# OpenHardware-Initiative/Drone-OA-IREE-ViT-Accelerator

Hardware: AMD Instinct MI355X
Metric: frames/s on ITAViTLSTM int8, 60x90 depth input (higher is better)
Workload: dtype int8+f32; 1 GPU; ITAViTLSTM int8 end-to-end forward (BASELINE config 4): 1024 synthetic 60x90 depth frames per GPU per step, LSTM state carried, velocity all-gather; frames_per_gpu=1024, global_batch=1024, parallelism=dp1, image_dtype=u8, weights=seed-0 synthetic QAT (tests/golden), gather_every=1, gather=none (one GPU), schedule=one stream

## Files before the change

### drone-oa-iree-vit-accelerator_amd/csrc/ita_lstm_head_kernel.h

```cpp
#pragma once
#include <cstddef>
#include "ita_f16x3_kernels.h"

__device__ __forceinline__ size_t ita_lstm_plane_index(int b, int k) {
  return ((size_t)(((b >> 5) * 4 + (k >> 6)) * 4 + ((k >> 4) & 3)) * 64 + ((k >> 3) & 1) * 32 + (b & 31)) * 8 + (k & 7);
}
__device__ __forceinline__ float lstm_sigmoid_fast(float x) {
  return __builtin_amdgcn_rcpf(1.0f + __builtin_amdgcn_exp2f(x * -1.44269504088896341f));
}
__device__ __forceinline__ float lstm_tanh_fast(float x) {
  return 1.0f - 2.0f * __builtin_amdgcn_rcpf(__builtin_amdgcn_exp2f(x * 2.88539008177792681f) + 1.0f);
}

__device__ __forceinline__ f32x16 mfma_f16x3(f32x16 acc, f16x8 wh, f16x8 wl, f16x8 xh, f16x8 xl) {
  acc = __builtin_amdgcn_mfma_f32_32x32x16_f16(wl, xh, acc, 0, 0, 0);
  acc = __builtin_amdgcn_mfma_f32_32x32x16_f16(wh, xl, acc, 0, 0, 0);
  return __builtin_amdgcn_mfma_f32_32x32x16_f16(wh, xh, acc, 0, 0, 0);
}
__device__ __forceinline__ void lstm_cell_fast(float gi, float gf, float gg, float go, float c_prev, float& c, float& h) {
  const float ig = lstm_sigmoid_fast(gi), fg = lstm_sigmoid_fast(gf), cg = lstm_tanh_fast(gg), og = lstm_sigmoid_fast(go);
  c = fmaf(fg, c_prev, ig * cg);
  h = og * lstm_tanh_fast(c);
}
__device__ __forceinline__ void split_f16x4(f32x4 x, f16x4& hi, f16x4& lo) {
#pragma unroll
  for (int j = 0; j < 4; ++j) {
    _Float16 a, b;
    split_f16(x[j], a, b);
    hi[j] = a;
    lo[j] = b;
  }
}
__device__ __forceinline__ f32x4 lstm_l0_extra(float dv, f32x4 q, int h, float& x4) {
  f32x4 x0 = {0.0f, 0.0f, 0.0f, 0.0f};
  x4 = 0.0f;
  if (h == 0) {
    x0 = (f32x4){dv / 10.0f, q.x, q.y, q.z};
    x4 = q.w;
  }
  return x0;
}
template <int NS>
__device__ __forceinline__ f32x4 sum_partials(const f32x4 (&pz)[NS]) {
  f32x4 ps = pz[0];
#pragma unroll
  for (int z = 1; z < NS; ++z) ps += pz[z];
  return ps;
}
__device__ __forceinline__ float lstm_sum4(const float (*part)[16][64], int e, int pl) {
  return ((part[0][e][pl] + part[1][e][pl]) + part[2][e][pl]) + part[3][e][pl];
}
template <class Live>
__device__ __forceinline__ void lstm_fc_rows(const float (*hs)[132], const float (*fw)[128], const float* fc_b, float* vel,
                                             size_t row0, int f0, int B, int tid, Live live) {
  if (tid < 96) {
    const int fr = tid / 3, o = tid - 3 * fr, b = f0 + fr;
    if (b < B && live(b)) {
      float acc = fc_b[o];
      for (int k = 0; k < 128; ++k) acc = fmaf(hs[fr][k], fw[o][k], acc);
      vel[(row0 + b) * 3 + o] = acc;
    }
  }
}

constexpr int ITA_HEAD_CNT_STRIDE = 64;
constexpr unsigned ITA_HEAD_ERR_TIMEOUT = 1;
constexpr unsigned long long ITA_HEAD_SPIN_TICKS = 200000000ull;
__device__ __forceinline__ void ita_store_sc1_f16x4(f16x4 v, __amdgpu_buffer_rsrc_t rsrc, int byte_off) {
  __builtin_amdgcn_raw_buffer_store_b64(__builtin_bit_cast(u32x2, v), rsrc, byte_off, 0, ITA_SC1);
}
__device__ __forceinline__ void ita_gather_h8(float hn, _Float16 (*pub)[32][8], int ef, int eu) {
  _Float16 x, y;
  split_f16(hn, x, y);
  pub[0][ef][eu] = x;
  pub[1][ef][eu] = y;
  __syncthreads();
}
__device__ __forceinline__ void ita_publish_h8(const _Float16 (*pub)[32][8], int r, __amdgpu_buffer_rsrc_t hi, int off_hi,
                                               __amdgpu_buffer_rsrc_t lo, int off_lo) {
  const f16x8 vh = *(const f16x8*)&pub[0][r][0], vl = *(const f16x8*)&pub[1][r][0];
  __builtin_amdgcn_raw_buffer_store_b128(__builtin_bit_cast(u32x4, vh), hi, off_hi, 0, ITA_SC1);
  __builtin_amdgcn_raw_buffer_store_b128(__builtin_bit_cast(u32x4, vl), lo, off_lo, 0, ITA_SC1);
}
__device__ __forceinline__ f16x8 ita_load_sc1_f16x8(__amdgpu_buffer_rsrc_t rsrc, int byte_off) {
  return __builtin_bit_cast(f16x8, __builtin_amdgcn_raw_buffer_load_b128(rsrc, byte_off, 0, ITA_SC1));
}
__device__ __forceinline__ f32x4 ita_load_sc1_f32x4(__amdgpu_buffer_rsrc_t rsrc, int byte_off) {
  return __builtin_bit_cast(f32x4, __builtin_amdgcn_raw_buffer_load_b128(rsrc, byte_off, 0, ITA_SC1));
}
__device__ __forceinline__ unsigned ita_head_arrive(unsigned* cnt, int ft, int tid) {
  asm volatile("s_waitcnt vmcnt(0)" ::: "memory");
  __syncthreads();
  unsigned prev = 0;
  if (tid == 0) prev = __hip_atomic_fetch_add(cnt + ft * ITA_HEAD_CNT_STRIDE, 1u, __ATOMIC_RELAXED, __HIP_MEMORY_SCOPE_AGENT);
  return prev;
}
__device__ __forceinline__ bool ita_head_poll(unsigned* cnt, unsigned target, unsigned* err) {
  const unsigned long long t0 = wall_clock64();
  while (__hip_atomic_load(cnt, __ATOMIC_RELAXED, __HIP_MEMORY_SCOPE_AGENT) < target) {
    if (wall_clock64() - t0 > ITA_HEAD_SPIN_TICKS) {
      __hip_atomic_fetch_or(err, ITA_HEAD_ERR_TIMEOUT, __ATOMIC_RELAXED, __HIP_MEMORY_SCOPE_AGENT);
      return false;
    }
    __builtin_amdgcn_s_sleep(2);
  }
  return true;
}


struct ItaLstmModelArgs {
  const float* part; float inv_fold_scale;
  const _Float16 *w0_hi, *w0_lo; float inv_wscale0;
  const float* bias0;
  const _Float16 *w1_hi, *w1_lo, *w2_hi, *w2_lo;
  float inv_wscale1, inv_wscale2;
  const float *bsum1, *bsum2;
};
struct ItaLstmHeadArgs {
  ItaLstmModelArgs m;
  const float *desvel, *quat;
  const float *h_in, *c_in;
  float *h_out, *c_out;
  size_t lstride;
  _Float16 *p1_hi, *p1_lo, *p2_hi, *p2_lo;
  const float *fc_w, *fc_b; float* vel;
  unsigned *cnt, *err;
  int B;
  const int* slots;
};
static_assert(sizeof(ItaLstmModelArgs) == 104 && offsetof(ItaLstmHeadArgs, desvel) == 104, "kernel-argument layout");

template <int NS>
__global__ __launch_bounds__(256, 2) void ita_lstm_head_kernel(const ItaLstmHeadArgs a) {
  __shared__ __attribute__((aligned(16))) float big[32 * 132 + 32 * 36];
  __shared__ __attribute__((aligned(16))) f16x8 hin[2][2][4][2][64];
  __shared__ __attribute__((aligned(16))) _Float16 pub[2][32][8];
  __shared__ unsigned flag;
  float (*hs)[132] = (float (*)[132])big;
  float (*pt)[36] = (float (*)[36])(big + 32 * 132);
  float (*part)[16][64] = (float (*)[16][64])big;
  const int tid = threadIdx.x, lane = tid & 63, wave = __builtin_amdgcn_readfirstlane(tid >> 6);
  const int ft = blockIdx.x >> 4, ut = blockIdx.x & 15, f0 = ft * 32;
  const int r = lane & 31, h = lane >> 5;
  const int B = a.B;
  const int ef = tid >> 3, eu = tid & 7;
  int rh[4], rb0 = min(f0 + r, B - 1), reb = min(f0 + ef, B - 1);
#pragma unroll
  for (int i = 0; i < 4; ++i) rh[i] = min(f0 + 2 * (4 * wave + i) + h, B - 1);
  if (a.slots) {
#pragma unroll
    for (int i = 0; i < 4; ++i) rh[i] = a.slots[rh[i]];
    rb0 = a.slots[rb0];
    reb = a.slots[reb];
  }

  f32x4 pz[NS];
#pragma unroll
  for (int z = 0; z < NS; ++z)
    pz[z] = *(const f32x4*)(a.m.part + ((size_t)z * B + min(f0 + 8 * wave + (lane >> 3), B - 1)) * 512 + ut * 32 + 4 * (lane & 7));
  f32x4 hv[4];
#pragma unroll
  for (int i = 0; i < 4; ++i) hv[i] = *(const f32x4*)(a.h_in + (size_t)rh[i] * 128 + 4 * r);
  const int b0 = f0 + r, u0 = ut * 8 + 4 * h;
  const size_t sb0 = (size_t)rb0;
  if (wave >= 2) {
    f32x4 hx[2][4][2];
#pragma unroll
    for (int l = 0; l < 2; ++l)
#pragma unroll
      for (int s = 0; s < 4; ++s) {
        const float* src = a.h_in + (l + 1) * a.lstride + sb0 * 128 + 64 * (wave - 2) + 16 * s + 8 * h;
        hx[l][s][0] = *(const f32x4*)src;
        hx[l][s][1] = *(const f32x4*)(src + 4);
      }
    __builtin_amdgcn_sched_barrier(0);
#pragma unroll
    for (int l = 0; l < 2; ++l)
#pragma unroll
      for (int s = 0; s < 4; ++s) {
        f16x8 xh, xl;
#pragma unroll
        for (int j = 0; j < 8; ++j) {
          _Float16 hi, lo;
          split_f16(hx[l][s][j >> 2][j & 3], hi, lo);
          xh[j] = hi;
          xl[j] = lo;
        }
        hin[l][wave - 2][s][0][lane] = xh;
        hin[l][wave - 2][s][1][lane] = xl;
      }
  }
  f16x8 wh[9], wl[9];
  f32x4 q = {0.0f, 0.0f, 0.0f, 0.0f}, ci0 = {0.0f, 0.0f, 0.0f, 0.0f}, bz[4];
  float dv = 0.0f;
  if (wave == 0) {
    const _Float16* wfr_hi = a.m.w0_hi + ((size_t)ut * 9 * 64 + lane) * 8;
    const _Float16* wfr_lo = a.m.w0_lo + ((size_t)ut * 9 * 64 + lane) * 8;
#pragma unroll
    for (int s = 0; s < 9; ++s) {
      wh[s] = *(const f16x8*)(wfr_hi + s * 512);
      wl[s] = *(const f16x8*)(wfr_lo + s * 512);
    }
    const int bc = min(b0, B - 1);
    q = *(const f32x4*)(a.quat + (size_t)bc * 4);
    dv = a.desvel[bc];
    ci0 = *(const f32x4*)(a.c_in + sb0 * 128 + u0);
#pragma unroll
    for (int gt = 0; gt < 4; ++gt) bz[gt] = *(const f32x4*)(a.m.bias0 + gt * 128 + u0);
  }
  const size_t wo = ((size_t)((ut * 4 + wave) * 4) * 64 + lane) * 8;
  f16x8 w1h[4], w1l[4];
#pragma unroll
  for (int s = 0; s < 4; ++s) {
    w1h[s] = *(const f16x8*)(a.m.w1_hi + wo + 512 * s);
    w1l[s] = *(const f16x8*)(a.m.w1_lo + wo + 512 * s);
  }
  const int eb = f0 + ef, un = ut * 8 + eu;
  const size_t esb = (size_t)reb;
  const float c1_prev = a.c_in[a.lstride + esb * 128 + un], c2_prev = a.c_in[2 * a.lstride + esb * 128 + un];
  float bs1[4], bs2[4];
#pragma unroll
  for (int gt = 0; gt < 4; ++gt) {
    bs1[gt] = a.m.bsum1[gt * 128 + un];
    bs2[gt] = a.m.bsum2[gt * 128 + un];
  }
  __builtin_amdgcn_sched_barrier(0);
  *(f32x4*)&pt[8 * wave + (lane >> 3)][4 * (lane & 7)] = sum_partials(pz);
#pragma unroll
  for (int i = 0; i < 4; ++i) *(f32x4*)&hs[2 * (4 * wave + i) + h][4 * r] = hv[i];
  __syncthreads();

  f32x4 hn0 = {0.0f, 0.0f, 0.0f, 0.0f};
  if (wave == 0) {
    f32x16 acc = {};
    float xlast1;
    const f32x4 xlast0 = lstm_l0_extra(dv, q, h, xlast1);
#pragma unroll
    for (int s = 0; s < 9; ++s) {
      f32x4 x0 = xlast0, x1 = {xlast1, 0.0f, 0.0f, 0.0f};
      if (s < 8) {
        x0 = *(const f32x4*)&hs[r][16 * s + 8 * h];
        x1 = *(const f32x4*)&hs[r][16 * s + 8 * h + 4];
      }
      f16x8 xh, xl;
#pragma unroll
      for (int j = 0; j < 8; ++j) {
        const float x = j < 4 ? x0[j & 3] : x1[j & 3];
        const _Float16 hi = (_Float16)x;
        xh[j] = hi;
        xl[j] = (_Float16)(x - (float)hi);
      }
      acc = mfma_f16x3(acc, wh[s], wl[s], xh, xl);
    }
    f32x4 cn;
#pragma unroll
    for (int q = 0; q < 4; ++q) {
      float g[4];
#pragma unroll
      for (int gt = 0; gt < 4; ++gt)
        g[gt] = (pt[r][gt * 8 + 4 * h + q] * a.m.inv_fold_scale + acc[4 * gt + q] * a.m.inv_wscale0) + bz[gt][q];
      float c, hn;
      lstm_cell_fast(g[0], g[1], g[2], g[3], ci0[q], c, hn);
      cn[q] = c;
      hn0[q] = hn;
    }
    if (b0 < B) *(f32x4*)(a.c_out + sb0 * 128 + u0) = cn;
    f16x4 x_hi, x_lo;
    split_f16x4(hn0, x_hi, x_lo);
    const int o0 = (int)ita_lstm_plane_index(b0, u0) * 2;
    ita_store_sc1_f16x4(x_hi, ita_rsrc(a.p1_hi), o0);
    ita_store_sc1_f16x4(x_lo, ita_rsrc(a.p1_lo), o0);
  }
  (void)ita_head_arrive(a.cnt, ft, tid);
  f16x8 w2h[4], w2l[4];
#pragma unroll
  for (int s = 0; s < 4; ++s) {
    w2h[s] = *(const f16x8*)(a.m.w2_hi + wo + 512 * s);
    w2l[s] = *(const f16x8*)(a.m.w2_lo + wo + 512 * s);
  }

#pragma unroll
  for (int l = 1; l <= 2; ++l) {
    if (tid == 0) flag = ita_head_poll(a.cnt + ft * ITA_HEAD_CNT_STRIDE, 16u * l, a.err) ? 1u : 0u;
    __syncthreads();
    if (!flag) return;
    if (l == 1 && wave == 0 && b0 < B) *(f32x4*)(a.h_out + sb0 * 128 + u0) = hn0;
    f16x8 fah[4], fal[4];
    if (wave < 2) {
      const int ao = (((ft * 4 + wave) * 4) * 64 + lane) * 16;
      const _Float16* ph = l == 1 ? a.p1_hi : a.p2_hi;
      const _Float16* pl = l == 1 ? a.p1_lo : a.p2_lo;
#pragma unroll
      for (int s = 0; s < 4; ++s) {
        fah[s] = ita_load_sc1_f16x8(ita_rsrc(ph), ao + 1024 * s);
        fal[s] = ita_load_sc1_f16x8(ita_rsrc(pl), ao + 1024 * s);
      }
    } else {
#pragma unroll
      for (int s = 0; s < 4; ++s) {
        fah[s] = hin[l - 1][wave - 2][s][0][lane];
        fal[s] = hin[l - 1][wave - 2][s][1][lane];
      }
    }
    f32x16 acc = {};
#pragma unroll
    for (int s = 0; s < 4; ++s) acc = mfma_f16x3(acc, l == 1 ? w1h[s] : w2h[s], l == 1 ? w1l[s] : w2l[s], fah[s], fal[s]);
#pragma unroll
    for (int e = 0; e < 16; ++e) part[wave][e][lane] = acc[e];
    __syncthreads();
    float gsum[4];
    const int pl = ef + 32 * (eu >> 2);
#pragma unroll
    for (int gte = 0; gte < 4; ++gte) gsum[gte] = lstm_sum4(part, 4 * gte + (eu & 3), pl);
    const float iws = l == 1 ? a.m.inv_wscale1 : a.m.inv_wscale2;
    const float* bs = l == 1 ? bs1 : bs2;
    const float gi = gsum[0] * iws + bs[0], gf = gsum[1] * iws + bs[1], gg = gsum[2] * iws + bs[2], go = gsum[3] * iws + bs[3];
    float c, hn;
    lstm_cell_fast(gi, gf, gg, go, l == 1 ? c1_prev : c2_prev, c, hn);
    const size_t so = l * a.lstride + esb * 128 + un;
    if (eb < B) {
      a.c_out[so] = c;
      if (l == 1) a.h_out[so] = hn;
      else
        __builtin_amdgcn_raw_buffer_store_b32(__builtin_bit_cast(unsigned, hn), ita_rsrc(a.h_out), (int)(so * 4), 0, ITA_SC1);
    }
    if (l == 1) {
      ita_gather_h8(hn, pub, ef, eu);
      if (wave == 0 && h == 0) {
        const int o = (int)ita_lstm_plane_index(f0 + r, ut * 8) * 2;
        ita_publish_h8(pub, r, ita_rsrc(a.p2_hi), o, ita_rsrc(a.p2_lo), o);
      }
    }
    const unsigned prev = ita_head_arrive(a.cnt, ft, tid);
    if (tid == 0 && l == 2) flag = prev == 47u ? 1u : 0u;
  }

  __syncthreads();
  if (!flag) return;
  if (tid == 0) __hip_atomic_store(a.cnt + ft * ITA_HEAD_CNT_STRIDE, 0u, __ATOMIC_RELAXED, __HIP_MEMORY_SCOPE_AGENT);
  float (*fw)[128] = (float (*)[128])(big + 32 * 132);
  int fro[4];
#pragma unroll
  for (int i = 0; i < 4; ++i) fro[i] = min(f0 + ((i * 256 + tid) >> 5), B - 1);
  if (a.slots) {
#pragma unroll
    for (int i = 0; i < 4; ++i) fro[i] = a.slots[fro[i]];
  }
  f32x4 hr[4];
#pragma unroll
  for (int i = 0; i < 4; ++i)
    hr[i] = ita_load_sc1_f32x4(ita_rsrc(a.h_out), (int)((2 * a.lstride + (size_t)fro[i] * 128 + 4 * (tid & 31)) * 4));
  const f32x4 wv = *(const f32x4*)(a.fc_w + 4 * min(tid, 95));
#pragma unroll
  for (int i = 0; i < 4; ++i) *(f32x4*)&hs[(i * 256 + tid) >> 5][4 * (tid & 31)] = hr[i];
  if (tid < 96) *(f32x4*)&fw[tid >> 5][4 * (tid & 31)] = wv;
  __syncthreads();
  lstm_fc_rows(hs, fw, a.fc_b, a.vel, 0, f0, B, tid, [](int) { return true; });
}
```

### drone-oa-iree-vit-accelerator_amd/csrc/ita_plugin.hip

```cpp
#include <hip/hip_runtime.h>

#include <algorithm>
#include <cstdio>
#include <cstdlib>
#include <cstring>
#include <mutex>
#include <string>
#include <atomic>
#include <thread>
#include <memory>
#include <type_traits>
#include <vector>

#include "../../include/ita_mi355x.h"
#include "../../include/ita_weights.h"
#include "../../include/ita_wire.h"
#include "ita_f16x3_kernels.h"
#include "ita_lstm_head_kernel.h"
#include "ita_lstm_seq_kernel.h"
#include "ita_f32_kernels.h"
#include "ita_int8_kernels.h"
#include "ita_stream_kernel.h"
#include "ita_long_attn_kernel.h"
#include "ita_long_stats_kernel.h"
// ... 1010 lines not shown
                                         (const float*)tp.row_max, (const float*)tp.row_sum, seq_len);
  });
}

}

int ita_mha_long_f32(ita_handle h, int layer, const float* x, float* y, int batch, int seq_len, void* stream) {
  if (int rc = check_layer_io(h, layer, x, y, batch)) return rc;
  return launch_long_f32(h, layer, x, y, false, batch, seq_len, (hipStream_t)stream);
}

int ita_mha_long_f32_taps(ita_handle h, int layer, const float* x, float* y, int batch, int seq_len,
                          const struct ita_mha_long_f32_taps* taps, void* stream) {
  if (int rc = check_layer_io(h, layer, x, y, batch)) return rc;
  const struct ita_mha_long_f32_taps none{};
  return launch_long_f32(h, layer, x, y, false, batch, seq_len, (hipStream_t)stream, taps ? taps : &none);
}

int ita_mha_long_f32_stats(ita_handle h, int layer, const float* x, int batch, int seq_len, float p_min,
                           const struct ita_mha_long_f32_stats* st, void* stream) {
  if (!h || !x || !st) return fail(ITA_ERR_INVALID_ARG, "null handle, x_dev or stats");
  if (!st->row_max && !st->row_sum && !st->row_gap && !st->row_nnz && !st->col_mass && !st->col_nnz)
    return fail(ITA_ERR_INVALID_ARG, "ita_mha_long_f32_stats: all six outputs are null");
  if (misaligned(st->row_max, 4) || misaligned(st->row_sum, 4) || misaligned(st->row_gap, 4) || misaligned(st->row_nnz, 4) ||
      misaligned(st->col_mass, 4) || misaligned(st->col_nnz, 4))
    return fail(ITA_ERR_INVALID_ARG, "every output must be 4-byte aligned");
  if (!(p_min > 0.0f && p_min <= 1.0f)) return fail(ITA_ERR_INVALID_ARG, "p_min must be in (0, 1]");
  if (int rc = check(h, batch)) return rc;
  if (layer < 0 || layer >= h->w.hdr.num_layers) return fail(ITA_ERR_INVALID_ARG, "bad layer");
  const Layer& L = h->w.layers[layer];
  hipStream_t s = (hipStream_t)stream;
  if (int rc = check_long_f32(L, batch, seq_len,
                              "this layer's attention is int8 (ITAW0001 / ITAW0002 blob): ita_mha_long_int8_stats reads it out")) return rc;
  const size_t nqt = (size_t)seq_len / 128, ntile = (size_t)batch * nqt;
  const size_t img = ntile * 2 * ItaLongF32Lds::UNIT, part = ntile * seq_len * 4;
  const bool cols = st->col_mass || st->col_nnz;
  if (int rc = ensure_long_f32_ws(h, 2 * img + (cols ? 2 * part : 0), s)) return rc;
  ItaLongF32Args a{};
  a.x = x;
  a.wk = L.wkf; a.wv = L.wvf; a.bk = L.bkf; a.bv = L.bvf;
  a.kimg = (f32x4*)(char*)h->long_ws; a.vimg = (f32x4*)((char*)h->long_ws + img);
  a.B = batch; a.S = seq_len;
  ItaLongF32StatsArgs sa{};
  sa.x = x; sa.wq = L.wqf; sa.bq = L.bqf; sa.kimg = a.kimg;
  sa.B = batch; sa.S = seq_len; sa.p_min = p_min;
  sa.row_max = st->row_max; sa.row_sum = st->row_sum; sa.row_gap = st->row_gap; sa.row_nnz = st->row_nnz;
  if (st->col_mass) sa.part_mass = (float*)((char*)h->long_ws + 2 * img);
  if (st->col_nnz) sa.part_nnz = (int*)((char*)h->long_ws + 2 * img + part);
  const size_t cap = 2 * (size_t)h->num_cus;
  const dim3 proj_grid((unsigned)(ntile < cap ? ntile : cap)), grid(seq_len / 128, batch);
  return with_E(h->w.hdr.E, [&](auto e) {
    constexpr int E = decltype(e)::value;
    if (int rc = launch<ita_lf32_proj_kernel<E>>(proj_grid, dim3(512), s, a)) return rc;
    if (int rc = launch<ita_lf32_stats_kernel<E>, ItaLongF32Lds::TOTAL>(grid, dim3(512), s, sa)) return rc;
    if (!cols) return (int)ITA_OK;
    const size_t n = (size_t)batch * seq_len, blocks = (n + 255) / 256;
    return launch<ita_lf32_colsum_kernel>(dim3(blocks < 4096 ? (unsigned)blocks : 4096u), dim3(256), s, (const float*)sa.part_mass,
                                          (const int*)sa.part_nnz, st->col_mass, st->col_nnz, (int)nqt, seq_len, n);
  });
}

int ita_encoder_layer_long_f32(ita_handle h, int layer, const float* x, float* y, int batch, int seq_len, void* stream) {
  if (int rc = check_layer_io(h, layer, x, y, batch)) return rc;
  const Layer& L = h->w.layers[layer];
  if (!L.ffn_f32) return fail(ITA_ERR_UNSUPPORTED, "this layer's FFN is int8 (ITAW0001 blob): ita_encoder_layer_long runs it");
  if (h->w.hdr.E != 64 && !L.w1p) return fail(ITA_ERR_UNSUPPORTED, "the float32 FFN of an ITAW0002 blob is built for E = 64");
  if (!L.attn_f32)
    if (int rc = check_long(L, batch, seq_len)) return rc;
  if (!L.n1w || !L.n2w) return fail(ITA_ERR_BAD_BLOB, "LayerNorm parameters missing from the blob");
  if (int rc = L.attn_f32 ? launch_long_f32(h, layer, x, y, true, batch, seq_len, (hipStream_t)stream)
                          : launch_long(h, layer, nullptr, nullptr, x, y, true, batch, seq_len, (hipStream_t)stream)) return rc;
  return launch_ffn_f32(h, layer, y, y, batch * (seq_len / 128), true, (hipStream_t)stream);
}

int ita_mha_q8(ita_handle h, int layer, const int8_t* x_q, int8_t* out_q, int batch, void* stream) {
  if (int rc = check_layer_io(h, layer, x_q, out_q, batch)) return rc;
  StreamIo io;
  io.xq = x_q; io.yq = out_q;
  return launch_stream(h, layer, 2, false, io, batch, (hipStream_t)stream);
}

int ita_ffn_int8_taps(ita_handle h, int layer, const float* x, float* y, int batch, const ita_ffn_taps* taps,
                      void* stream) {
  if (int rc = check_layer_io(h, layer, x, y, batch)) return rc;
  return launch_ffn(h, layer, x, y, batch, false, taps, (hipStream_t)stream);
}
int ita_ffn_int8(ita_handle h, int layer, const float* x, float* y, int batch, void* stream) {
  return ita_ffn_int8_taps(h, layer, x, y, batch, nullptr, stream);
}

int ita_get_ffn_kind(ita_handle h, int layer, int* kind) {
  if (!h || !h->w.loaded) return fail(ITA_ERR_NO_WEIGHTS, "no weights loaded");
  if (!kind || layer < 0 || layer >= h->w.hdr.num_layers) return fail(ITA_ERR_INVALID_ARG, "bad pointer or layer");
  *kind = h->w.layers[layer].ffn_f32 ? ITA_FFN_F32 : ITA_FFN_INT8;
  return ITA_OK;
}

int ita_ffn_f32(ita_handle h, int layer, const float* x, float* y, int batch, void* stream) {
  if (int rc = check_layer_io(h, layer, x, y, batch)) return rc;
  return launch_ffn_f32(h, layer, x, y, batch, false, (hipStream_t)stream);
}

static_assert(ITA_HEAD_ERR_TIMEOUT == ITA_HEAD_TIMEOUT, "one error code, two names");
int ita_head_status(ita_handle h, int* status) {
  int rc = check(h, 1, false);
  if (rc) return rc;
  if (!status) return fail(ITA_ERR_INVALID_ARG, "null pointer");
  *status = 0;
  if (!h->ws.head_sync) return ITA_OK;
  unsigned v = 0;
  HIPCHK(hipDeviceSynchronize());
  HIPCHK(hipMemcpy(&v, h->ws.head_sync, sizeof(v), hipMemcpyDeviceToHost));
  if (v) {
    HIPCHK(hipMemset(h->ws.head_sync, 0, h->ws.head_sync_bytes));
    HIPCHK(hipDeviceSynchronize());
  }
  *status = (int)v;
  return ITA_OK;
}

int ita_get_attn_kind(ita_handle h, int layer, int* kind) {
  if (!h || !h->w.loaded) return fail(ITA_ERR_NO_WEIGHTS, "no weights loaded");
  if (!kind || layer < 0 || layer >= h->w.hdr.num_layers) return fail(ITA_ERR_INVALID_ARG, "bad pointer or layer");
  *kind = h->w.layers[layer].attn_f32 ? ITA_ATTN_F32 : ITA_ATTN_INT8;
  return ITA_OK;
}

int ita_mha_f32(ita_handle h, int layer, const float* x, float* y, int batch, void* stream) {
  if (int rc = check_layer_io(h, layer, x, y, batch)) return rc;
  return launch_attn_f32(h, layer, x, y, batch, false, (hipStream_t)stream);
}

int ita_encoder_layer(ita_handle h, int layer, const float* x, float* y, int batch, void* stream) {
  if (int rc = check_layer_io(h, layer, x, y, batch)) return rc;
  StreamIo io;
  io.x = x; io.y = y;
  return launch_encoder(h, layer, io, batch, (hipStream_t)stream);
}

int ita_debug_encoder_stamps(ita_handle h, int layer, const float* x, const void* image_u8, float* y, int batch,
                             unsigned long long* stamps, void* stream) {
  int rc = check(h, batch);
  if (rc) return rc;
  if ((!x && !image_u8) || !y || !stamps || layer < 0 || layer >= h->w.hdr.num_layers)
    return fail(ITA_ERR_INVALID_ARG, "bad argument");
  if (h->w.layers[layer].attn_f32) return fail(ITA_ERR_UNSUPPORTED, "this layer's attention is float32 (ITAW0003 blob): no stream kernel, no stamps");
  if (image_u8 ? !h->w.layers[layer].simg_tok : !h->w.layers[layer].simg_enc)
    return fail(ITA_ERR_UNSUPPORTED, "this layer does not run on the stream kernel");
  StreamIo io;
  io.x = x; io.y = y; io.stamps = stamps; io.img = image_u8;
  return launch_encoder(h, layer, io, batch, (hipStream_t)stream);
}

#ifdef ITA_UP_STAMP
int ita_debug_tail_up_stamps(unsigned long long* host_dst, int count) {
  if (hipDeviceSynchronize() != hipSuccess) return ITA_ERR_HIP;
  return hipMemcpyFromSymbol(host_dst, HIP_SYMBOL(ita_up_stamp_buf), sizeof(unsigned long long) * (size_t)count) == hipSuccess ? ITA_OK : ITA_ERR_HIP;
}
#endif
int ita_debug_softmax_rows(ita_handle h, const int8_t* logits, uint8_t* probs, int rows, void* stream) {
  int rc = check(h, rows, false);
  if (rc) return rc;
  if (!logits || !probs) return fail(ITA_ERR_INVALID_ARG, "null pointer");
  return launch<ita_softmax_rows_kernel>(dim3((rows + 15) / 16), dim3(64), (hipStream_t)stream, logits, probs, rows);
}

int ita_debug_fast_site_ok(float mult) { return fast_site_ok(mult) ? 1 : 0; }

int ita_debug_layer_forms(ita_handle h, int layer, unsigned* fast_sites, int* stream_images) {
  if (!h || !h->w.loaded) return fail(ITA_ERR_NO_WEIGHTS, "no weights loaded");
  if (!fast_sites || !stream_images || layer < 0 || layer >= h->w.hdr.num_layers)
    return fail(ITA_ERR_INVALID_ARG, "bad pointer or layer");
  const Layer& L = h->w.layers[layer];
  *fast_sites = L.fast_sites;
  *stream_images = (L.simg_mha ? ITA_FORMS_ATTN_IMAGE : 0) | (L.simg_enc ? ITA_FORMS_LAYER_IMAGE : 0) |
                       (L.simg_tok ? ITA_FORMS_TOK_IMAGE : 0);
  return ITA_OK;
}

int ita_tokenizer(ita_handle h, const void* image, int image_dtype, float* tokens, int batch, void* stream) {
  int rc = check(h, batch);
  if (rc) return rc;
  if (!image || !tokens || (image_dtype != ITA_IMAGE_F32 && image_dtype != ITA_IMAGE_U8))
    return fail(ITA_ERR_INVALID_ARG, "bad pointer or image dtype");
  return launch_tokenizer(h, image, image_dtype, tokens, batch, (hipStream_t)stream);
}

int ita_ingest(ita_handle h, const void* src, int pixel_dtype, int height, int width, long long row_stride,
               long long frame_stride, float depth_scale, float* frames, int batch, void* stream) {
  if (!h) return fail(ITA_ERR_INVALID_ARG, "null handle");
  if (!src || !frames) return fail(ITA_ERR_INVALID_ARG, "null pointer");
  if (pixel_dtype != ITA_PIXEL_U8 && pixel_dtype != ITA_PIXEL_U16 && pixel_dtype != ITA_PIXEL_F32)
    return fail(ITA_ERR_INVALID_ARG, "pixel_dtype must be ITA_PIXEL_U8, ITA_PIXEL_U16 or ITA_PIXEL_F32");
  if (int rc = check_frames(height, width, row_stride, frame_stride, batch)) return rc;
  const size_t px = pixel_dtype == ITA_PIXEL_U8 ? 1 : pixel_dtype == ITA_PIXEL_U16 ? 2 : 4;
  if ((uintptr_t)src % px || (uintptr_t)frames % sizeof(float))
    return fail(ITA_ERR_INVALID_ARG, "src must be aligned to its pixel size, frames to 4 bytes");
  if (pixel_dtype == ITA_PIXEL_U16 && !(depth_scale > 0.0f && depth_scale <= 3.402823466e38f))
    return fail(ITA_ERR_INVALID_ARG, "depth_scale must be finite and positive");
  HIPCHK(hipSetDevice(h->device));
  hipStream_t s = (hipStream_t)stream;
  switch (pixel_dtype) {
    case ITA_PIXEL_U8: return launch_ingest<uint8_t>(h, src, height, width, row_stride, frame_stride, depth_scale, frames, batch, s);
    case ITA_PIXEL_U16: return launch_ingest<uint16_t>(h, src, height, width, row_stride, frame_stride, depth_scale, frames, batch, s);
    default: return launch_ingest<float>(h, src, height, width, row_stride, frame_stride, depth_scale, frames, batch, s);
  }
}

int ita_tokenizer_long(ita_handle h, const void* src, int pixel_dtype, int height, int width, long long row_stride,
                       long long frame_stride, float depth_scale, int tok_h, int tok_w, float* tokens, int batch, void* stream) {
  if (!h) return fail(ITA_ERR_INVALID_ARG, "null handle");
  if (!src || !tokens) return fail(ITA_ERR_INVALID_ARG, "null pointer");
  if (pixel_dtype != ITA_PIXEL_U8 && pixel_dtype != ITA_PIXEL_U16 && pixel_dtype != ITA_PIXEL_F32)
    return fail(ITA_ERR_INVALID_ARG, "pixel_dtype must be ITA_PIXEL_U8, ITA_PIXEL_U16 or ITA_PIXEL_F32");
  if (int rc = check_frames(height, width, row_stride, frame_stride, batch)) return rc;
  const size_t px = pixel_dtype == ITA_PIXEL_U8 ? 1 : pixel_dtype == ITA_PIXEL_U16 ? 2 : 4;
  if ((uintptr_t)src % px || (uintptr_t)tokens % 16)
    return fail(ITA_ERR_INVALID_ARG, "src must be aligned to its pixel size, tokens to 16 bytes");
  if (pixel_dtype == ITA_PIXEL_U16 && !(depth_scale > 0.0f && depth_scale <= 3.402823466e38f))
    return fail(ITA_ERR_INVALID_ARG, "depth_scale must be finite and positive");
  if (tok_h < 1 || tok_w < 16 || tok_w % 16 || tok_w > 65536 || (long long)tok_h * tok_w % 128 || (long long)tok_h * tok_w > 65536 ||
      batch > 65535)
    return fail(ITA_ERR_UNSUPPORTED, "needs tok_h >= 1, tok_w % 16 == 0, tok_h * tok_w a multiple of 128 up to 65536, batch <= 65535");
  if (!h->w.loaded) return fail(ITA_ERR_NO_WEIGHTS, "ita_load_weights has not been called");
  if (!h->w.tok_simg) return fail(ITA_ERR_BAD_BLOB, "tokenizer parameters missing from the blob");
  HIPCHK(hipSetDevice(h->device));
  hipStream_t s = (hipStream_t)stream;
  StageRecorder rec(h, s, false);
  int rc = rec.mark(0, false);
  if (rc) return rc;
  switch (pixel_dtype) {
    case ITA_PIXEL_U8: rc = launch_tokenizer_long<uint8_t>(h, src, height, width, row_stride, frame_stride, depth_scale, tok_h, tok_w, tokens, batch, s); break;
    case ITA_PIXEL_U16: rc = launch_tokenizer_long<uint16_t>(h, src, height, width, row_stride, frame_stride, depth_scale, tok_h, tok_w, tokens, batch, s); break;
    default: rc = launch_tokenizer_long<float>(h, src, height, width, row_stride, frame_stride, depth_scale, tok_h, tok_w, tokens, batch, s);
  }
  if (rc || (rc = rec.mark(0, true))) return rc;
  rec.finish();
  return ITA_OK;
}

int ita_resize_table(int n_in, int n_out, int* n0, int* count, float* coeff, int coeff_width, int* width_out) {
  if (!n0 || !count || !coeff || !width_out || coeff_width < 1) return fail(ITA_ERR_INVALID_ARG, "null pointer or coeff_width < 1");
  ItaResizeAxis t;
  if (!ita_resize_axis(n_in, n_out, t)) return fail(ITA_ERR_INVALID_ARG, "n_in must be in [1, 4096], n_out in [1, 4096]");
  *width_out = t.width;
  if (t.width > coeff_width) return fail(ITA_ERR_INVALID_ARG, "coeff_width is smaller than the table's width (see width_out)");
  for (int o = 0; o < n_out; ++o) {
    n0[o] = t.n0[o];
    count[o] = t.count[o];
    for (int j = 0; j < coeff_width; ++j) coeff[(size_t)o * coeff_width + j] = j < t.width ? t.coeff[(size_t)o * t.width + j] : 0.0f;
  }
  return ITA_OK;
}

int ita_ingest_wire_prepare(ita_handle h, int height, int width) {
  if (!h) return fail(ITA_ERR_INVALID_ARG, "null handle");
  if (height < 1 || height > ITA_WIRE_MAX_DIM || width < 1 || width > ITA_WIRE_MAX_DIM)
    return fail(ITA_ERR_INVALID_ARG, "height and width must be in [1, 4096]");
  HIPCHK(hipSetDevice(h->device));
  return prepare_wire(h, height, width, nullptr);
}

int ita_ingest_wire(ita_handle h, const uint8_t* src, int height, int width, long long row_stride, long long frame_stride,
                    uint8_t* wire, int batch, void* stream) {
  if (!h) return fail(ITA_ERR_INVALID_ARG, "null handle");
  if (!src || !wire) return fail(ITA_ERR_INVALID_ARG, "null pointer");
  if (int rc = check_frames(height, width, row_stride, frame_stride, batch)) return rc;
  HIPCHK(hipSetDevice(h->device));
  hipStream_t s = (hipStream_t)stream;
  WireSize* w = find_wire(h, height, width);
  if (!w) {
    if (capturing(s))
      return fail(ITA_ERR_INVALID_ARG, "this source size has no tables yet and they cannot be built inside a stream capture; call ita_ingest_wire_prepare first");
    const int rc = prepare_wire(h, height, width, &w);
    if (rc) return rc;
  }
  int rows = 4, span = 0;
  if (row_stride % 4 == 0)
    for (int b = 2; b >= 0 && !span; --b)
      if (ita_wire_lds_bytes(width, w->span[b]) <= ITA_WIRE_STAGED_LDS_MAX) {
        rows = 4 * (b + 1);
        span = w->span[b];
      }
  const long long items = (long long)batch * ((ITA_WIRE_H + rows - 1) / rows);
  const int grid = (int)std::min<long long>(items, (long long)h->num_cus * 8);
  const int lds = ita_wire_lds_bytes(width, span);
  auto run = [&](auto dwords, auto staged) {
    constexpr bool DWORDS = decltype(dwords)::value, STAGED = decltype(staged)::value;
    return launch_lds<ita_ingest_wire_kernel<DWORDS, STAGED>, STAGED ? ITA_WIRE_STAGED_LDS_MAX : 0>(
        dim3(grid), dim3(256), lds, s, src, height, width, row_stride, frame_stride, w->dev, wire, batch, rows, span);
  };
  if (span) return run(std::true_type{}, std::true_type{});
  if (row_stride % 4 == 0) return run(std::true_type{}, std::false_type{});
  return run(std::false_type{}, std::false_type{});
}

int ita_fusion_tail(ita_handle h, const float* x, float* feat, int batch, void* stream) {
  int rc = check(h, batch);
  if (rc) return rc;
  if (!x || !feat) return fail(ITA_ERR_INVALID_ARG, "null pointer");
  return launch_tail(h->num_cus, h->w.hdr.E, h->w.tail_wT, h->w.tail_b, x, feat, 4608, batch, (hipStream_t)stream);
}

int ita_fusion_tail_load(ita_handle h, const float* conv_w, const float* conv_b, int E, int out_ch) {
  int rc = check(h, 1, false);
  if (rc) return rc;
// ... 521 lines not shown
```

Before: 11.54 million frames/s.

## Move layer-1/2 h_in split into global planes, defer W1/W2 register loads

Drops the shared-memory hin staging that waves 2-3 used to hold the previous-step hidden state for layers 1 and 2. Wave 1 now splits its slice of the prior h into hi/lo f16 and writes it straight into the global p1/p2 plane buffers, so every wave reads its MFMA operands from those planes. W1 weights are loaded after the first arrive and W2 only after layer 1 finishes, reusing one register set, which cuts register pressure and LDS use. Compile-time timestamp instrumentation is added behind ITA_HEAD_STAMP; it is off by default.

```diff
diff --git a/drone-oa-iree-vit-accelerator_amd/csrc/ita_lstm_head_kernel.h b/drone-oa-iree-vit-accelerator_amd/csrc/ita_lstm_head_kernel.h
--- a/drone-oa-iree-vit-accelerator_amd/csrc/ita_lstm_head_kernel.h
+++ b/drone-oa-iree-vit-accelerator_amd/csrc/ita_lstm_head_kernel.h
@@ -130,10 +130,19 @@
 };
 static_assert(sizeof(ItaLstmModelArgs) == 104 && offsetof(ItaLstmHeadArgs, desvel) == 104, "kernel-argument layout");
 
+#ifdef ITA_HEAD_STAMP
+constexpr int ITA_HEAD_NSTAMP = 12;
+__device__ unsigned long long ita_head_stamp_buf[2048 * ITA_HEAD_NSTAMP];
+#define ITA_HEAD_ST(i) do { __builtin_amdgcn_sched_barrier(0); st[i] = __builtin_amdgcn_s_memrealtime(); __builtin_amdgcn_sched_barrier(0); } while (0)
+#define ITA_HEAD_ST_FLUSH() do { if (tid == 0 && blockIdx.x < 2048) _Pragma("unroll") for (int i_ = 0; i_ < ITA_HEAD_NSTAMP; ++i_) ita_head_stamp_buf[(size_t)blockIdx.x * ITA_HEAD_NSTAMP + i_] = st[i_]; } while (0)
+#else
+#define ITA_HEAD_ST(i) do {} while (0)
+#define ITA_HEAD_ST_FLUSH() do {} while (0)
+#endif
+
 template <int NS>
 __global__ __launch_bounds__(256, 2) void ita_lstm_head_kernel(const ItaLstmHeadArgs a) {
   __shared__ __attribute__((aligned(16))) float big[32 * 132 + 32 * 36];
-  __shared__ __attribute__((aligned(16))) f16x8 hin[2][2][4][2][64];
   __shared__ __attribute__((aligned(16))) _Float16 pub[2][32][8];
   __shared__ unsigned flag;
   float (*hs)[132] = (float (*)[132])big;
@@ -143,6 +152,10 @@
   const int ft = blockIdx.x >> 4, ut = blockIdx.x & 15, f0 = ft * 32;
   const int r = lane & 31, h = lane >> 5;
   const int B = a.B;
+#ifdef ITA_HEAD_STAMP
+  unsigned long long st[ITA_HEAD_NSTAMP] = {};
+#endif
+  ITA_HEAD_ST(0);
   const int ef = tid >> 3, eu = tid & 7;
   int rh[4], rb0 = min(f0 + r, B - 1), reb = min(f0 + ef, B - 1);
 #pragma unroll
@@ -163,32 +176,11 @@
   for (int i = 0; i < 4; ++i) hv[i] = *(const f32x4*)(a.h_in + (size_t)rh[i] * 128 + 4 * r);
   const int b0 = f0 + r, u0 = ut * 8 + 4 * h;
   const size_t sb0 = (size_t)rb0;
-  if (wave >= 2) {
-    f32x4 hx[2][4][2];
-#pragma unroll
-    for (int l = 0; l < 2; ++l)
-#pragma unroll
-      for (int s = 0; s < 4; ++s) {
-        const float* src = a.h_in + (l + 1) * a.lstride + sb0 * 128 + 64 * (wave - 2) + 16 * s + 8 * h;
-        hx[l][s][0] = *(const f32x4*)src;
-        hx[l][s][1] = *(const f32x4*)(src + 4);
-      }
-    __builtin_amdgcn_sched_barrier(0);
-#pragma unroll
-    for (int l = 0; l < 2; ++l)
-#pragma unroll
-      for (int s = 0; s < 4; ++s) {
-        f16x8 xh, xl;
-#pragma unroll
-        for (int j = 0; j < 8; ++j) {
-          _Float16 hi, lo;
-          split_f16(hx[l][s][j >> 2][j & 3], hi, lo);
-          xh[j] = hi;
-          xl[j] = lo;
-        }
-        hin[l][wave - 2][s][0][lane] = xh;
-        hin[l][wave - 2][s][1][lane] = xl;
-      }
+  f32x4 hx0 = {0.0f, 0.0f, 0.0f, 0.0f}, hx1 = hx0;
+  if (wave == 1) {
+    const float* src = a.h_in + (h + 1) * a.lstride + sb0 * 128 + ut * 8;
+    hx0 = *(const f32x4*)src;
+    hx1 = *(const f32x4*)(src + 4);
   }
   f16x8 wh[9], wl[9];
   f32x4 q = {0.0f, 0.0f, 0.0f, 0.0f}, ci0 = {0.0f, 0.0f, 0.0f, 0.0f}, bz[4];
@@ -208,13 +200,6 @@
 #pragma unroll
     for (int gt = 0; gt < 4; ++gt) bz[gt] = *(const f32x4*)(a.m.bias0 + gt * 128 + u0);
   }
-  const size_t wo = ((size_t)((ut * 4 + wave) * 4) * 64 + lane) * 8;
-  f16x8 w1h[4], w1l[4];
-#pragma unroll
-  for (int s = 0; s < 4; ++s) {
-    w1h[s] = *(const f16x8*)(a.m.w1_hi + wo + 512 * s);
-    w1l[s] = *(const f16x8*)(a.m.w1_lo + wo + 512 * s);
-  }
   const int eb = f0 + ef, un = ut * 8 + eu;
   const size_t esb = (size_t)reb;
   const float c1_prev = a.c_in[a.lstride + esb * 128 + un], c2_prev = a.c_in[2 * a.lstride + esb * 128 + un];
@@ -225,10 +210,14 @@
     bs2[gt] = a.m.bsum2[gt * 128 + un];
   }
   __builtin_amdgcn_sched_barrier(0);
-  *(f32x4*)&pt[8 * wave + (lane >> 3)][4 * (lane & 7)] = sum_partials(pz);
+  ITA_HEAD_ST(1);
+  const f32x4 psum = sum_partials(pz);
+  ITA_HEAD_ST(2);
+  *(f32x4*)&pt[8 * wave + (lane >> 3)][4 * (lane & 7)] = psum;
 #pragma unroll
   for (int i = 0; i < 4; ++i) *(f32x4*)&hs[2 * (4 * wave + i) + h][4 * r] = hv[i];
   __syncthreads();
+  ITA_HEAD_ST(3);
 
   f32x4 hn0 = {0.0f, 0.0f, 0.0f, 0.0f};
   if (wave == 0) {
@@ -271,12 +260,32 @@
     ita_store_sc1_f16x4(x_hi, ita_rsrc(a.p1_hi), o0);
     ita_store_sc1_f16x4(x_lo, ita_rsrc(a.p1_lo), o0);
   }
+  if (wave == 1) {
+    f16x8 xh, xl;
+#pragma unroll
+    for (int j = 0; j < 8; ++j) {
+      _Float16 hi, lo;
+      split_f16(j < 4 ? hx0[j & 3] : hx1[j & 3], hi, lo);
+      xh[j] = hi;
+      xl[j] = lo;
+    }
+    const int o = (int)ita_lstm_plane_index(f0 + r, 128 + ut * 8) * 2;
+    if (h == 0) {
+      __builtin_amdgcn_raw_buffer_store_b128(__builtin_bit_cast(u32x4, xh), ita_rsrc(a.p1_hi), o, 0, ITA_SC1);
+      __builtin_amdgcn_raw_buffer_store_b128(__builtin_bit_cast(u32x4, xl), ita_rsrc(a.p1_lo), o, 0, ITA_SC1);
+    } else {
+      __builtin_amdgcn_raw_buffer_store_b128(__builtin_bit_cast(u32x4, xh), ita_rsrc(a.p2_hi), o, 0, ITA_SC1);
+      __builtin_amdgcn_raw_buffer_store_b128(__builtin_bit_cast(u32x4, xl), ita_rsrc(a.p2_lo), o, 0, ITA_SC1);
+    }
+  }
   (void)ita_head_arrive(a.cnt, ft, tid);
-  f16x8 w2h[4], w2l[4];
+  ITA_HEAD_ST(4);
+  const size_t wo = ((size_t)((ut * 4 + wave) * 4) * 64 + lane) * 8;
+  f16x8 wlh[4], wll[4];
 #pragma unroll
   for (int s = 0; s < 4; ++s) {
-    w2h[s] = *(const f16x8*)(a.m.w2_hi + wo + 512 * s);
-    w2l[s] = *(const f16x8*)(a.m.w2_lo + wo + 512 * s);
+    wlh[s] = *(const f16x8*)(a.m.w1_hi + wo + 512 * s);
+    wll[s] = *(const f16x8*)(a.m.w1_lo + wo + 512 * s);
   }
 
 #pragma unroll
@@ -284,9 +293,10 @@
     if (tid == 0) flag = ita_head_poll(a.cnt + ft * ITA_HEAD_CNT_STRIDE, 16u * l, a.err) ? 1u : 0u;
     __syncthreads();
     if (!flag) return;
+    ITA_HEAD_ST(3 + 2 * l);
     if (l == 1 && wave == 0 && b0 < B) *(f32x4*)(a.h_out + sb0 * 128 + u0) = hn0;
     f16x8 fah[4], fal[4];
-    if (wave < 2) {
+    {
       const int ao = (((ft * 4 + wave) * 4) * 64 + lane) * 16;
       const _Float16* ph = l == 1 ? a.p1_hi : a.p2_hi;
       const _Float16* pl = l == 1 ? a.p1_lo : a.p2_lo;
@@ -295,16 +305,10 @@
         fah[s] = ita_load_sc1_f16x8(ita_rsrc(ph), ao + 1024 * s);
         fal[s] = ita_load_sc1_f16x8(ita_rsrc(pl), ao + 1024 * s);
       }
-    } else {
-#pragma unroll
-      for (int s = 0; s < 4; ++s) {
-        fah[s] = hin[l - 1][wave - 2][s][0][lane];
-        fal[s] = hin[l - 1][wave - 2][s][1][lane];
-      }
     }
     f32x16 acc = {};
 #pragma unroll
-    for (int s = 0; s < 4; ++s) acc = mfma_f16x3(acc, l == 1 ? w1h[s] : w2h[s], l == 1 ? w1l[s] : w2l[s], fah[s], fal[s]);
+    for (int s = 0; s < 4; ++s) acc = mfma_f16x3(acc, wlh[s], wll[s], fah[s], fal[s]);
 #pragma unroll
     for (int e = 0; e < 16; ++e) part[wave][e][lane] = acc[e];
     __syncthreads();
@@ -332,11 +336,22 @@
       }
     }
     const unsigned prev = ita_head_arrive(a.cnt, ft, tid);
+    ITA_HEAD_ST(4 + 2 * l);
+    if (l == 1) {
+#pragma unroll
+      for (int s = 0; s < 4; ++s) {
+        wlh[s] = *(const f16x8*)(a.m.w2_hi + wo + 512 * s);
+        wll[s] = *(const f16x8*)(a.m.w2_lo + wo + 512 * s);
+      }
+    }
     if (tid == 0 && l == 2) flag = prev == 47u ? 1u : 0u;
   }
 
   __syncthreads();
-  if (!flag) return;
+  if (!flag) {
+    ITA_HEAD_ST_FLUSH();
+    return;
+  }
   if (tid == 0) __hip_atomic_store(a.cnt + ft * ITA_HEAD_CNT_STRIDE, 0u, __ATOMIC_RELAXED, __HIP_MEMORY_SCOPE_AGENT);
   float (*fw)[128] = (float (*)[128])(big + 32 * 132);
   int fro[4];
@@ -356,4 +371,9 @@
   if (tid < 96) *(f32x4*)&fw[tid >> 5][4 * (tid & 31)] = wv;
   __syncthreads();
   lstm_fc_rows(hs, fw, a.fc_b, a.vel, 0, f0, B, tid, [](int) { return true; });
-}
+#ifdef ITA_HEAD_STAMP
+  asm volatile("s_waitcnt vmcnt(0)" ::: "memory");
+#endif
+  ITA_HEAD_ST(9);
+  ITA_HEAD_ST_FLUSH();
+}
diff --git a/drone-oa-iree-vit-accelerator_amd/csrc/ita_plugin.hip b/drone-oa-iree-vit-accelerator_amd/csrc/ita_plugin.hip
--- a/drone-oa-iree-vit-accelerator_amd/csrc/ita_plugin.hip
+++ b/drone-oa-iree-vit-accelerator_amd/csrc/ita_plugin.hip
@@ -1186,6 +1186,12 @@
   return launch_encoder(h, layer, io, batch, (hipStream_t)stream);
 }
 
+#ifdef ITA_HEAD_STAMP
+int ita_debug_head_stamps(unsigned long long* host_dst, int count) {
+  if (hipDeviceSynchronize() != hipSuccess) return ITA_ERR_HIP;
+  return hipMemcpyFromSymbol(host_dst, HIP_SYMBOL(ita_head_stamp_buf), sizeof(unsigned long long) * (size_t)count) == hipSuccess ? ITA_OK : ITA_ERR_HIP;
+}
+#endif
 #ifdef ITA_UP_STAMP
 int ita_debug_tail_up_stamps(unsigned long long* host_dst, int count) {
   if (hipDeviceSynchronize() != hipSuccess) return ITA_ERR_HIP;
```

Result: no change. 11.60 million frames/s (median of 6 runs) (+0.5%).
